# jbush001/RustNetworkStack

Hardware: AMD Instinct MI355X
Metric: GiB/s device-resident Internet checksum, 1500B-packet batches, 1/2/4/8 GPUs (higher is better)
Workload: dtype u8

## Files before the change

rustnetworkstack_amd/csrc/k_shapes.hip:

```cpp
#include "rns_launch.hpp"

namespace rns {

template <int G, int U, bool S>
int launch_shape(const CsumArgs &a, uint32_t variant, uint32_t max_blocks, hipStream_t st)
{
    uint64_t blocks;
    if ((variant & 5) == 0) {
        constexpr uint32_t kGroups = kBlock / G;
        blocks = (static_cast<uint64_t>(a.n) + kGroups - 1) / kGroups;
    } else {
        const uint64_t batches = waves64(a.n);
        const uint64_t wpb = ((variant & 4) ? kMixedBlock<false> : kBlock) / 64;
        blocks = (batches + wpb - 1) / wpb;
    }
    if (max_blocks != 0 && blocks > max_blocks)
        blocks = max_blocks;
    if (blocks == 0)
        return RNS_OK;
    const dim3 grid(static_cast<uint32_t>(blocks)), block((variant & 4) ? kMixedBlock<false> : kBlock);
    const bool nt = (variant & 2) != 0;
    const uint32_t cap = (variant >> 8) & 15u;
    const size_t lds = cap ? ((160u << 10) / cap) - (2u << 10) : 0u;
    variant &= 0xffu;
    if ((variant & 5) == 0) {
        if constexpr (G >= 4)
            return with_flags([&](auto NT) { return launch(csum_batch_kernel<G, U, S, NT()>, grid, block, lds, st, a); },
                              nt);
        return RNS_E_INVALID;
    }
    return with_flags(
        [&](auto NT, auto BUF) {
            if (variant & 4)
                return launch(csum_mixed_kernel<S, NT(), BUF(), false>, grid, block, lds, st, a);
            if constexpr (G <= 8 && U <= 2) {
                if (variant & 8)
                    return launch(csum_rounds_kernel<G, U, S, NT(), BUF(), G>, grid, block, lds, st, a);
                if (variant & 16)
                    return launch(csum_rounds_kernel<G, U, S, NT(), BUF(), 1, false, true>, grid, block, lds, st, a);
            } else if (variant & 24) {
                return static_cast<int>(RNS_E_INVALID);
            }
            return launch(csum_rounds_kernel<G, U, S, NT(), BUF()>, grid, block, lds, st, a);
        },
        nt, buf_ok(a));
}

template <bool S>
int dispatch(const CsumArgs &a, uint32_t variant, uint32_t G, uint32_t U, uint32_t max_blocks, hipStream_t st)
{
    const uint32_t v = variant & 0xffu;
    if (v > 31 || (variant >> 12) || ((v & 24) && (v & 5) != 1) || (v & 24) == 24)
        return RNS_E_INVALID;
    if (variant & 4)
        return launch_shape<64, 4, S>(a, variant, max_blocks, st);
#define RNS_SHAPE(g, u) \
    if (G == g && U == u) return launch_shape<g, u, S>(a, variant, max_blocks, st);
    if (variant & 1) {
        RNS_SHAPE(2, 1) RNS_SHAPE(2, 2) RNS_SHAPE(2, 4)
    }
    RNS_SHAPE(4, 1) RNS_SHAPE(4, 2) RNS_SHAPE(4, 4) RNS_SHAPE(4, 8)
    RNS_SHAPE(8, 1) RNS_SHAPE(8, 2) RNS_SHAPE(8, 4) RNS_SHAPE(8, 8)
    RNS_SHAPE(16, 1) RNS_SHAPE(16, 2) RNS_SHAPE(16, 4) RNS_SHAPE(16, 8)
    RNS_SHAPE(32, 1) RNS_SHAPE(32, 2) RNS_SHAPE(32, 4) RNS_SHAPE(32, 8)
    RNS_SHAPE(64, 1) RNS_SHAPE(64, 2) RNS_SHAPE(64, 4) RNS_SHAPE(64, 8)
#undef RNS_SHAPE
    return RNS_E_INVALID;
}

template int dispatch<false>(const CsumArgs &, uint32_t, uint32_t, uint32_t, uint32_t, hipStream_t);
template int dispatch<true>(const CsumArgs &, uint32_t, uint32_t, uint32_t, uint32_t, hipStream_t);

int launch_strided_tiny(const CsumArgs &a, hipStream_t st)
{
    constexpr int B = 2;
    const dim3 grid(static_cast<uint32_t>((static_cast<uint64_t>(a.n) + 64 * B - 1) / (64 * B))), block(64);
    return with_flags([&](auto buf) { return launch(csum_strided_tiny_kernel<buf(), B>, grid, block, 0, st, a); },
                      buf_ok(a));
}

}
```

rustnetworkstack_amd/csrc/rns_checksum.hip:

```cpp
#include <hip/hip_runtime.h>

#include <algorithm>
#include <cmath>
#include <cstdint>
#include <cstdio>

#include "rns_launch.hpp"

using namespace rns;

namespace {

__global__ __launch_bounds__(kBlock) void splitmix64_fill_kernel(uint8_t *buf, uint64_t nbytes, uint64_t seed)
{
    const uint64_t nwords = (nbytes + 7) / 8;
    const uint64_t stride = static_cast<uint64_t>(gridDim.x) * blockDim.x;
    for (uint64_t i = static_cast<uint64_t>(blockIdx.x) * blockDim.x + threadIdx.x; i < nwords; i += stride) {
        uint64_t z = seed + (i + 1) * 0x9E3779B97F4A7C15ull;
        z = (z ^ (z >> 30)) * 0xBF58476D1CE4E5B9ull;
        z = (z ^ (z >> 27)) * 0x94D049BB133111EBull;
        z = z ^ (z >> 31);
        if ((i + 1) * 8 <= nbytes) {
            reinterpret_cast<uint64_t *>(buf)[i] = z;
        } else {
            for (uint64_t b = i * 8; b < nbytes; ++b)
                buf[b] = static_cast<uint8_t>(z >> (8 * (b - i * 8)));
        }
    }
}

template <class Body>
int entry(uint32_t n, bool valid, const uint8_t *d_arena, uint64_t arena_bytes, uint32_t flags, void *stream, Body body)
{
    if (n == 0)
        return RNS_OK;
    if (!d_arena || !valid)
        return RNS_E_INVALID;
    if (int st = check_device())
        return st;
    CsumArgs a{};
    set_arena(a, d_arena, arena_bytes);
    a.n = n;
    a.flags = flags;
    return body(a, static_cast<hipStream_t>(stream));
}

void set_explicit(CsumArgs &a, const uint64_t *d_off, const uint32_t *d_len)
{
    a.off = d_off;
    a.len = d_len;
}

void set_packed(CsumArgs &a, const uint64_t *d_blk_off, const uint16_t *d_len16, uint32_t align_log2)
{
    a.len16 = d_len16;
    a.blk_off = d_blk_off;
    a.align_mask = (1u << align_log2) - 1u;
}

bool packed_align(uint32_t align_log2, uint32_t lo) { return align_log2 >= lo && align_log2 <= 12; }

void set_strided(CsumArgs &a, uint64_t first_off, uint64_t stride)
{
    a.first_off = first_off;
    a.stride = stride;
}

bool strided_fits(uint64_t first_off, uint64_t stride, uint32_t n)
{
    const uint64_t room = ~0ull - 16u - first_off;
    return first_off <= ~0ull - 16u && (n <= 1 || stride <= room / (n - 1));
}

void set_chain(CsumArgs &a, const uint64_t *d_frag_off, const uint32_t *d_frag_len, const uint32_t *d_first,
               uint32_t n_frags)
{
    a.off = d_frag_off;
    a.len = d_frag_len;
    a.first = d_first;
    a.n_frags = n_frags;
}

static_assert(RNS_CHAIN_MAX_PACKETS == 0xFFFFFFFFu - 64u * kChainMaxK, "rns_checksum.h's chain cap");
bool chain_valid(const uint64_t *d_frag_off, const uint32_t *d_frag_len, const uint32_t *d_first, uint32_t n_frags,
                 uint32_t n_pkts)
{
    return d_first && (!n_frags || (d_frag_off && d_frag_len)) && n_pkts <= RNS_CHAIN_MAX_PACKETS;
}

void set_results(CsumArgs &a, const uint16_t *d_seed, uint16_t *d_out, uint32_t *d_bad)
{
    a.seed = d_seed;
    a.out = d_out;
    a.bad = d_bad;
}

void set_field(CsumArgs &a, const uint16_t *d_field, uint32_t field_off)
{
    a.field = d_field;
    a.field_off = field_off;
}

uint32_t be_sum(const uint8_t *p, int nbytes)
{
    uint32_t s = 0;
    for (int k = 0; k < nbytes; k += 2)
        s += static_cast<uint32_t>(p[k]) << 8 | p[k + 1];
    return s;
}

void set_rx(CsumArgs &a, uint8_t *d_status, uint16_t *d_l4_sum, const uint8_t *local_ipv4, const uint8_t *local_ipv6)
{
    a.status = d_status;
    a.l4_out = d_l4_sum;
    a.local4_sum = be_sum(local_ipv4, 4);
    a.local6_sum = be_sum(local_ipv6, 16);
}

bool rx_valid(const uint8_t *d_status, const uint8_t *local_ipv4, const uint8_t *local_ipv6)
{
    return d_status && local_ipv4 && local_ipv6;
}

void set_tx_status(CsumArgs &a, uint8_t *d_status) { a.status = d_status; }

uint32_t chain_pick_k(double mean)
{
    uint32_t K = 1;
    double best = -1.0;
    for (uint32_t k = 1; k <= kChainMaxK; ++k) {
        const double fr = k * mean, fill = fr > 0 ? fr / std::ceil(fr) : 1.0;
        if (fill > best + 0.02) {
            best = fill;
            K = k;
        }
    }
    return K;
}

double chain_mean(const CsumArgs &a) { return static_cast<double>(a.n_frags) / static_cast<double>(a.n); }

#ifndef RNS_CHAIN_NT_FROM
#define RNS_CHAIN_NT_FROM 384u
#endif
bool chain_nt_from_hint(uint32_t frag_len_hint) { return (frag_len_hint ? frag_len_hint : 512u) >= RNS_CHAIN_NT_FROM; }
bool chain_nt_from_arena(uint64_t arena_bytes, uint32_t n_frags, double mean)
{
    const double frag_est = mean > 0.5 ? static_cast<double>(arena_bytes) / n_frags * (mean - 0.5) / mean : 0.0;
    return n_frags == 0 || frag_est >= RNS_CHAIN_NT_FROM;
}

bool chain_deep(uint32_t K, double mean) { return K >= 3 || (K == 2 && mean >= 2.0); }

template <bool FILL>
int chain_launch(CsumArgs &a, uint32_t frag_len_hint, hipStream_t stream)
{
    const double mean = chain_mean(a);
    a.chain_k = chain_pick_k(mean);
    if ((a.flags & RNS_FLAG_CHAIN_TX_PACKED) && mean <= 1.0 + kRunFrags)
        return launch_txrows<FILL>(a, stream);
    const bool runs = kChainRuns && (a.flags & RNS_FLAG_CHAIN_RUNS) && buf_ok(a);
    return launch_chain<FILL>(a, a.chain_k, chain_nt_from_hint(frag_len_hint), runs, chain_deep(a.chain_k, mean), stream);
}

constexpr uint64_t kRxGridCap = 4096;
dim3 stash_grid(uint64_t n, uint64_t arena_bytes, bool tiny_cap)
{
    constexpr int BLK = kMixedBlock<true>;
    uint64_t blocks = (waves64(n) + BLK / 64 - 1) / (BLK / 64);
    const bool cap = tiny_cap && arena_bytes / n <= 128;
    if (cap && blocks > kRxGridCap)
        blocks = kRxGridCap;
    return dim3(static_cast<uint32_t>(blocks));
}

}

extern "C" {

int rns_csum_batch_dev_cfg(const uint8_t *d_arena, uint64_t arena_bytes, const uint64_t *d_off,
                           const uint32_t *d_len, const uint16_t *d_seed, uint16_t *d_out, uint32_t n,
                           uint32_t flags, uint32_t variant, uint32_t lanes_per_packet, uint32_t unroll,
                           uint32_t max_blocks, uint32_t *d_bad, void *stream)
{
    return entry(n, d_off && d_len && d_out, d_arena, arena_bytes, flags, stream, [&](CsumArgs &a, hipStream_t st) {
        set_explicit(a, d_off, d_len);
        set_results(a, d_seed, d_out, d_bad);
        return dispatch<false>(a, variant, lanes_per_packet, unroll, max_blocks, st);
    });
}

int rns_csum_batch_dev(const uint8_t *d_arena, uint64_t arena_bytes, const uint64_t *d_off,
                       const uint32_t *d_len, const uint16_t *d_seed, uint16_t *d_out, uint32_t n,
                       uint32_t flags, uint32_t len_hint, uint32_t *d_bad, void *stream)
{
    const Shape sh = pick_shape(len_hint);
    return rns_csum_batch_dev_cfg(d_arena, arena_bytes, d_off, d_len, d_seed, d_out, n, flags, sh.variant, sh.G,
                                  sh.U, sh.max_blocks, d_bad, stream);
}

int rns_csum_batch_dev_off32(const uint8_t *d_arena, uint64_t arena_bytes, const uint32_t *d_off32,
                             const uint32_t *d_len, const uint16_t *d_seed, uint16_t *d_out, uint32_t n,
                             uint32_t flags, uint32_t len_hint, uint32_t *d_bad, void *stream)
{
    return entry(n, d_off32 && d_len && d_out, d_arena, arena_bytes, flags, stream, [&](CsumArgs &a, hipStream_t st) {
        a.off32 = d_off32;
        a.len = d_len;
        set_results(a, d_seed, d_out, d_bad);
        const Shape sh = pick_shape(len_hint);
        return dispatch<false>(a, sh.variant, sh.G, sh.U, sh.max_blocks, st);
    });
}

int rns_csum_batch_packed_dev(const uint8_t *d_arena, uint64_t arena_bytes, const uint64_t *d_blk_off,
                              const uint16_t *d_len16, uint32_t align_log2, const uint16_t *d_seed, uint16_t *d_out,
                              uint32_t n, uint32_t flags, uint32_t len_hint, uint32_t *d_bad, void *stream)
{
    return entry(n, d_blk_off && d_len16 && d_out && packed_align(align_log2, 0), d_arena, arena_bytes, flags, stream,
                 [&](CsumArgs &a, hipStream_t st) {
                     set_packed(a, d_blk_off, d_len16, align_log2);
                     set_results(a, d_seed, d_out, d_bad);
                     a.len_hint = len_hint;
                     Shape sh = pick_shape(len_hint);
                     if ((sh.variant & 5u) == 0)
                         sh = Shape{6u, 0u, 0u, 0u};
                     return dispatch_packed(a, sh, st);
                 });
}

int rns_csum_batch_strided_dev(const uint8_t *d_arena, uint64_t arena_bytes, uint64_t first_off,
                               uint64_t stride, uint32_t len, const uint16_t *d_seed, uint16_t *d_out,
                               uint32_t n, uint32_t flags, uint32_t *d_bad, void *stream)
{
    return entry(n, d_out && strided_fits(first_off, stride, n), d_arena, arena_bytes, flags, stream,
                 [&](CsumArgs &a, hipStream_t st) {
                     set_strided(a, first_off, stride);
                     set_results(a, d_seed, d_out, d_bad);
                     a.fixed_len = len;
                     if (len != 0 && len <= 64 && ((first_off + a.base_adjust) & 15) == 0 && (stride & 15) == 0)
                         return launch_strided_tiny(a, st);
                     const Shape sh = pick_shape(len);
                     return dispatch<true>(a, sh.variant, sh.G, sh.U, sh.max_blocks, st);
                 });
}

int rns_csum_chain_dev(const uint8_t *d_arena, uint64_t arena_bytes, const uint64_t *d_frag_off,
                       const uint32_t *d_frag_len, uint32_t n_frags, const uint32_t *d_first,
                       const uint16_t *d_seed, uint16_t *d_out, uint32_t n_pkts, uint32_t flags,
                       uint32_t frag_len_hint, uint16_t *d_frag_sums, uint32_t *d_bad, void *stream)
{
    (void)d_frag_sums;
    return entry(n_pkts, d_out && chain_valid(d_frag_off, d_frag_len, d_first, n_frags, n_pkts), d_arena, arena_bytes,
                 flags, stream, [&](CsumArgs &a, hipStream_t st) {
                     set_chain(a, d_frag_off, d_frag_len, d_first, n_frags);
                     set_results(a, d_seed, d_out, d_bad);
                     return chain_launch<false>(a, frag_len_hint, st);
                 });
}

int rns_csum_chain_fill_dev(uint8_t *d_arena, uint64_t arena_bytes, const uint64_t *d_frag_off,
                            const uint32_t *d_frag_len, uint32_t n_frags, const uint32_t *d_first,
                            const uint16_t *d_seed, const uint16_t *d_field, uint32_t field_off, uint16_t *d_out,
                            uint32_t n_pkts, uint32_t flags, uint32_t frag_len_hint, uint32_t *d_bad, void *stream)
{
    return entry(n_pkts, chain_valid(d_frag_off, d_frag_len, d_first, n_frags, n_pkts), d_arena, arena_bytes, flags,
                 stream, [&](CsumArgs &a, hipStream_t st) {
                     set_chain(a, d_frag_off, d_frag_len, d_first, n_frags);
                     set_results(a, d_seed, d_out, d_bad);
                     set_field(a, d_field, field_off);
                     return chain_launch<true>(a, frag_len_hint, st);
                 });
}

int rns_csum_fill_dev(uint8_t *d_arena, uint64_t arena_bytes, const uint64_t *d_off, const uint32_t *d_len,
                      const uint16_t *d_seed, const uint16_t *d_field, uint32_t field_off, uint16_t *d_out,
                      uint32_t n, uint32_t flags, uint32_t *d_bad, void *stream)
{
    return entry(n, d_off && d_len, d_arena, arena_bytes, flags, stream, [&](CsumArgs &a, hipStream_t st) {
        set_explicit(a, d_off, d_len);
        set_results(a, d_seed, d_out, d_bad);
        set_field(a, d_field, field_off);
        return launch_fill(a, stash_grid(n, arena_bytes, false), st);
    });
}

int rns_csum_fill_packed_dev(uint8_t *d_arena, uint64_t arena_bytes, const uint64_t *d_blk_off, const uint16_t *d_len16,
                             uint32_t align_log2, const uint16_t *d_seed, const uint16_t *d_field, uint32_t field_off,
                             uint16_t *d_out, uint32_t n, uint32_t flags, uint32_t len_hint, uint32_t *d_bad,
                             void *stream)
{
    return entry(n, d_blk_off && d_len16 && packed_align(align_log2, 4), d_arena, arena_bytes, flags, stream,
                 [&](CsumArgs &a, hipStream_t st) {
                     set_packed(a, d_blk_off, d_len16, align_log2);
                     set_results(a, d_seed, d_out, d_bad);
                     set_field(a, d_field, field_off);
                     a.len_hint = len_hint;
                     return launch_fill_packed(a, st);
                 });
}

int rns_rx_verify_dev(const uint8_t *d_arena, uint64_t arena_bytes, const uint64_t *d_off, const uint32_t *d_len,
                      uint32_t n, const uint8_t *local_ipv4, const uint8_t *local_ipv6, uint8_t *d_status,
                      uint16_t *d_l4_sum, void *stream)
{
    return entry(n, d_off && d_len && rx_valid(d_status, local_ipv4, local_ipv6), d_arena, arena_bytes,
                 RNS_FLAG_COMPLEMENT, stream, [&](CsumArgs &a, hipStream_t st) {
                     set_explicit(a, d_off, d_len);
                     set_rx(a, d_status, d_l4_sum, local_ipv4, local_ipv6);
                     return launch_rx(a, stash_grid(n, arena_bytes, true), st);
                 });
}

int rns_rx_verify_packed_dev(const uint8_t *d_arena, uint64_t arena_bytes, const uint64_t *d_blk_off,
                             const uint16_t *d_len16, uint32_t align_log2, uint32_t n, const uint8_t *local_ipv4,
                             const uint8_t *local_ipv6, uint8_t *d_status, uint16_t *d_l4_sum, void *stream)
{
    return entry(n, d_blk_off && d_len16 && rx_valid(d_status, local_ipv4, local_ipv6) && packed_align(align_log2, 4),
                 d_arena, arena_bytes, RNS_FLAG_COMPLEMENT, stream, [&](CsumArgs &a, hipStream_t st) {
                     set_packed(a, d_blk_off, d_len16, align_log2);
                     set_rx(a, d_status, d_l4_sum, local_ipv4, local_ipv6);
                     return launch_stream_rx(a, st);
                 });
}

int rns_rx_verify_strided_dev(const uint8_t *d_arena, uint64_t arena_bytes, uint64_t first_off, uint64_t stride,
                              const uint16_t *d_len16, uint32_t n, const uint8_t *local_ipv4, const uint8_t *local_ipv6,
                              uint8_t *d_status, uint16_t *d_l4_sum, void *stream)
{
    return entry(n, d_len16 && rx_valid(d_status, local_ipv4, local_ipv6) && strided_fits(first_off, stride, n), d_arena,
                 arena_bytes, RNS_FLAG_COMPLEMENT, stream, [&](CsumArgs &a, hipStream_t st) {
                     a.len16 = d_len16;
                     set_strided(a, first_off, stride);
                     set_rx(a, d_status, d_l4_sum, local_ipv4, local_ipv6);
                     return launch_strided_rx(a, st);
                 });
}

int rns_rx_verify_chain_dev(const uint8_t *d_arena, uint64_t arena_bytes, const uint64_t *d_frag_off,
                            const uint32_t *d_frag_len, uint32_t n_frags, const uint32_t *d_first, uint32_t n_pkts,
                            const uint8_t *local_ipv4, const uint8_t *local_ipv6, uint8_t *d_status, uint16_t *d_l4_sum,
                            void *stream)
{
    return entry(n_pkts,
                 chain_valid(d_frag_off, d_frag_len, d_first, n_frags, n_pkts) &&
                     rx_valid(d_status, local_ipv4, local_ipv6),
                 d_arena, arena_bytes, RNS_FLAG_COMPLEMENT, stream, [&](CsumArgs &a, hipStream_t st) {
                     set_chain(a, d_frag_off, d_frag_len, d_first, n_frags);
                     set_rx(a, d_status, d_l4_sum, local_ipv4, local_ipv6);
                     const double mean = chain_mean(a);
                     a.chain_k = chain_pick_k(mean);
                     return launch_rx_chain(a, a.chain_k, chain_nt_from_arena(arena_bytes, n_frags, mean), st);
                 });
}

int rns_rx_verify_pool_dev(const uint8_t *d_pool, uint64_t pool_bytes, uint32_t buf_log2, const uint32_t *d_buf_idx,
                           uint32_t n_frags, const uint32_t *d_blk_first, const uint16_t *d_len16, uint32_t n_pkts,
                           const uint8_t *local_ipv4, const uint8_t *local_ipv6, uint8_t *d_status, uint16_t *d_l4_sum,
                           void *stream)
{
    return entry(n_pkts,
                 buf_log2 >= kPoolMinLog2 && buf_log2 <= kPoolMaxLog2 && d_blk_first && d_len16 &&
                     (!n_frags || d_buf_idx) && n_pkts <= RNS_CHAIN_MAX_PACKETS &&
                     (reinterpret_cast<uintptr_t>(d_pool) & 15) == 0 && rx_valid(d_status, local_ipv4, local_ipv6),
                 d_pool, pool_bytes, RNS_FLAG_COMPLEMENT, stream, [&](CsumArgs &a, hipStream_t st) {
                     a.off32 = d_buf_idx;
                     a.n_frags = n_frags;
                     a.first = d_blk_first;
                     a.len16 = d_len16;
                     a.align_mask = (1u << buf_log2) - 1u;
                     set_rx(a, d_status, d_l4_sum, local_ipv4, local_ipv6);
                     const double mean = chain_mean(a);
                     a.chain_k = chain_pick_k(mean);
                     return launch_rx_pool(a, a.chain_k, chain_nt_from_arena(pool_bytes, n_frags, mean), st);
                 });
}

int rns_tx_fill_packed_dev(uint8_t *d_arena, uint64_t arena_bytes, const uint64_t *d_blk_off, const uint16_t *d_len16,
                           uint32_t align_log2, uint32_t n, uint8_t *d_status, uint32_t len_hint, void *stream)
{
    return entry(n, d_blk_off && d_len16 && packed_align(align_log2, 4), d_arena, arena_bytes, RNS_FLAG_COMPLEMENT,
                 stream, [&](CsumArgs &a, hipStream_t st) {
                     set_packed(a, d_blk_off, d_len16, align_log2);
                     set_tx_status(a, d_status);
                     a.len_hint = len_hint;
                     return launch_tx_packed(a, st);
                 });
}

int rns_tx_fill_chain_dev(uint8_t *d_arena, uint64_t arena_bytes, const uint64_t *d_frag_off, const uint32_t *d_frag_len,
                          uint32_t n_frags, const uint32_t *d_first, uint32_t n_pkts, uint8_t *d_status, void *stream)
{
    return entry(n_pkts, chain_valid(d_frag_off, d_frag_len, d_first, n_frags, n_pkts), d_arena, arena_bytes,
                 RNS_FLAG_COMPLEMENT, stream, [&](CsumArgs &a, hipStream_t st) {
                     set_chain(a, d_frag_off, d_frag_len, d_first, n_frags);
                     set_tx_status(a, d_status);
                     return launch_txrows<false, true>(a, st);
                 });
}

int rns_tx_fill_chain_packed_dev(uint8_t *d_arena, uint64_t arena_bytes, const uint64_t *d_head_blk_off,
                                 const uint8_t *d_head_len8, const uint64_t *d_pay_blk_off, const uint16_t *d_pay_len16,
                                 uint32_t pay_align_log2, uint32_t n, uint8_t *d_status, void *stream)
{
    return entry(n,
                 d_head_blk_off && d_head_len8 && d_pay_blk_off && d_pay_len16 && packed_align(pay_align_log2, 4) &&
                     n <= RNS_CHAIN_MAX_PACKETS,
                 d_arena, arena_bytes, RNS_FLAG_COMPLEMENT, stream, [&](CsumArgs &a, hipStream_t st) {
                     a.head_blk_off = d_head_blk_off;
                     a.head_len8 = d_head_len8;
                     set_packed(a, d_pay_blk_off, d_pay_len16, pay_align_log2);
                     set_tx_status(a, d_status);
                     return launch_txrows<false, true, true>(a, st);
                 });
}

int rns_tx_fill_dev(uint8_t *d_arena, uint64_t arena_bytes, const uint64_t *d_off, const uint32_t *d_len,
                    uint32_t n, uint8_t *d_status, void *stream)
{
    return entry(n, d_off && d_len, d_arena, arena_bytes, RNS_FLAG_COMPLEMENT, stream, [&](CsumArgs &a, hipStream_t st) {
        set_explicit(a, d_off, d_len);
        set_tx_status(a, d_status);
        return launch_tx(a, stash_grid(n, arena_bytes, true), st);
    });
}

int rns_fill_splitmix64_dev(uint8_t *d_buf, uint64_t nbytes, uint64_t seed, void *stream)
{
    if (nbytes == 0)
        return RNS_OK;
    if (!d_buf || (reinterpret_cast<uintptr_t>(d_buf) & 7))
        return RNS_E_INVALID;
    if (int st = check_device())
        return st;
    const uint64_t words = (nbytes + 7) / 8;
    const uint32_t blocks = static_cast<uint32_t>(std::min<uint64_t>((words + kBlock - 1) / kBlock, 8192));
    hipLaunchKernelGGL(splitmix64_fill_kernel, dim3(blocks), dim3(kBlock), 0, static_cast<hipStream_t>(stream),
                       d_buf, nbytes, seed);
    return hip_status(hipGetLastError());
}

const char *rns_csum_shape_name(uint32_t len_hint)
{
    static const char *const names[] = {"csum_batch_kernel",     "csum_rounds_kernel",     "csum_batch_kernel[nt]",
                                        "csum_rounds_kernel[nt]", "csum_mixed_kernel",      "csum_mixed_kernel",
                                        "csum_mixed_kernel[nt]",  "csum_mixed_kernel[nt]"};
    static thread_local char buf[96];
    const Shape sh = pick_shape(len_hint);
    if (sh.variant & 4)
        std::snprintf(buf, sizeof(buf), "%s (size classes G/U 4/1 x 4 packets, 4/4, 16/4, 32/4, 64/4)", names[sh.variant & 7]);
    else
        std::snprintf(buf, sizeof(buf), "%s<G=%u,U=%u>%s%s", names[sh.variant & 7], sh.G, sh.U,
                      (sh.variant & 8) ? " all rounds in flight" : (sh.variant & 16) ? " descriptors prefetched" : "",
                      sh.max_blocks ? " grid-capped" : "");
    return buf;
}

const char *rns_build_info(void)
{
    return "rns_checksum abi=1 offload-arch=gfx950 kernels=csum_rows_kernel (packed form: 1 KiB rows per 64-packet "
           "region, owners capture two region prefixes and sum their own end chunk; fill mode), csum_rows_rx_kernel "
           "(packed receive verify: the rows plus each owner's header chunks loaded a group ahead), csum_stream_kernel "
           "(receive verify of ACK-sized arenas: owners load their datagrams whole), csum_strided_rx_kernel (receive "
           "verify of fixed-size slots: quad-coalesced rows), csum_rows_tx_kernel (packed transmit finalize through the "
           "rows), csum_txrows_kernel (transmit-shaped chains: packed payload rows + owner-loaded head fragments; "
           "head-fragment fill; whole finalize of NetBuffer chains with the heads written back from LDS), "
           "csum_strided_tiny_kernel "
           "(fixed-size packets <= 64 B at a fixed stride), csum_mixed_kernel (per-wave size-class sort; verify / fill / "
           "transmit-finalize stash modes), csum_rounds_kernel, csum_batch_kernel, csum_chain_kernel (one pass, "
           "per-fragment fold; head-fragment fill) (v_sad_u16 LE sums, v_dot4 BE sums past 128 KiB, wave64, DPP "
           "reductions)";
}

int rns_device_count(void)
{
    int n = 0;
    if (hipGetDeviceCount(&n) != hipSuccess) {
        (void)hipGetLastError();
        return 0;
    }
    return n;
}

}
```

rustnetworkstack_amd/csrc/rns_kernels.hpp:

```cpp
#pragma once

#include "rns_k_common.hpp"
#include "rns_k_rounds.hpp"
#include "rns_k_mixed.hpp"
#include "rns_k_chain.hpp"
#include "rns_k_chain_rx.hpp"
#include "rns_k_pool_rx.hpp"
#include "rns_k_stream.hpp"
#include "rns_k_rows.hpp"
#include "rns_k_rows_rx.hpp"
#include "rns_k_rows_tx.hpp"
#include "rns_k_txrows.hpp"
```

rustnetworkstack_amd/csrc/rns_launch.hpp:

```cpp
#pragma once

#include <type_traits>

#include "rns_kernels.hpp"

namespace rns {

inline int hip_status(hipError_t e) { return e == hipSuccess ? RNS_OK : RNS_E_HIP_BASE - static_cast<int>(e); }

struct Shape {
    uint32_t variant, G, U, max_blocks;
};

constexpr uint32_t kTinyVariant = 19u;
constexpr uint32_t kTinyGrid = 2048u;
inline Shape pick_shape(uint32_t len_hint)
{
    const uint32_t chunks = len_hint ? (len_hint + 15) / 16 + 1 : 96;
    if (chunks <= 8)
        return Shape{kTinyVariant, 4u, 1u, kTinyGrid};
    if (chunks <= 48)
        return Shape{4u, 0u, 0u, 0u};
    if (chunks <= 160)
        return Shape{6u, 0u, 0u, 0u};
    return Shape{2u, 64u, 4u, 0u};
}

inline int check_device()
{
    int n = 0;
    if (hipGetDeviceCount(&n) != hipSuccess || n <= 0) {
        (void)hipGetLastError();
        return RNS_E_NODEVICE;
    }
    return RNS_OK;
}

inline void set_arena(CsumArgs &a, const uint8_t *arena, uint64_t arena_bytes)
{
    const uintptr_t p = reinterpret_cast<uintptr_t>(arena);
    a.base_adjust = p & 15;
    a.arena = reinterpret_cast<const uint8_t *>(p - a.base_adjust);
    a.arena_bytes = arena_bytes + a.base_adjust;
}

inline bool buf_ok(const CsumArgs &a) { return buf_records(a) < kOobOffset; }

inline uint32_t waves64(uint64_t n) { return static_cast<uint32_t>((n + 63) / 64); }

template <class F>
int with_flags(F &&f)
{
    return f();
}
template <class F, class... Rest>
int with_flags(F &&f, bool b, Rest... rest)
{
    auto bind = [&](auto c) { return with_flags([&](auto... cs) { return f(c, cs...); }, rest...); };
    return b ? bind(std::true_type{}) : bind(std::false_type{});
}

template <uint32_t KM, uint32_t... More, class F>
int with_kmax(uint32_t K, F &&f)
{
    if constexpr (sizeof...(More) == 0)
        return f(std::integral_constant<uint32_t, KM>{});
    else
        return K <= KM ? f(std::integral_constant<uint32_t, KM>{}) : with_kmax<More...>(K, f);
}

inline int launch(void (*kernel)(const CsumArgs), dim3 grid, dim3 block, size_t lds, hipStream_t st, const CsumArgs &a)
{
    hipLaunchKernelGGL(kernel, grid, block, lds, st, a);
    return hip_status(hipGetLastError());
}

template <bool S>
int dispatch(const CsumArgs &a, uint32_t variant, uint32_t G, uint32_t U, uint32_t max_blocks, hipStream_t st);
extern template int dispatch<false>(const CsumArgs &, uint32_t, uint32_t, uint32_t, uint32_t, hipStream_t);
extern template int dispatch<true>(const CsumArgs &, uint32_t, uint32_t, uint32_t, uint32_t, hipStream_t);
int launch_strided_tiny(const CsumArgs &a, hipStream_t st);
int dispatch_packed(const CsumArgs &a, const Shape &sh, hipStream_t st);
int launch_fill_packed(const CsumArgs &a, hipStream_t st);
int launch_stream_rx(const CsumArgs &a, hipStream_t st);
int launch_tx_packed(const CsumArgs &a, hipStream_t st);
int launch_strided_rx(const CsumArgs &a, hipStream_t st);
template <bool FILL>
int launch_chain(const CsumArgs &a, uint32_t K, bool nt, bool runs, bool deep, hipStream_t st);
extern template int launch_chain<false>(const CsumArgs &, uint32_t, bool, bool, bool, hipStream_t);
extern template int launch_chain<true>(const CsumArgs &, uint32_t, bool, bool, bool, hipStream_t);
template <bool FILL, bool FIN = false, bool CPT = false>
int launch_txrows(const CsumArgs &a, hipStream_t st);
extern template int launch_txrows<false, false, false>(const CsumArgs &, hipStream_t);
extern template int launch_txrows<true, false, false>(const CsumArgs &, hipStream_t);
extern template int launch_txrows<false, true, false>(const CsumArgs &, hipStream_t);
extern template int launch_txrows<false, true, true>(const CsumArgs &, hipStream_t);
int launch_rx_chain(const CsumArgs &a, uint32_t K, bool nt, hipStream_t st);
int launch_rx_pool(const CsumArgs &a, uint32_t K, bool nt, hipStream_t st);
int launch_fill(const CsumArgs &a, dim3 grid, hipStream_t st);
int launch_rx(const CsumArgs &a, dim3 grid, hipStream_t st);
int launch_tx(const CsumArgs &a, dim3 grid, hipStream_t st);

}
```

rustnetworkstack_amd/csrc/rns_pipeline.hip:

```cpp
#include <hip/hip_runtime.h>

#include <algorithm>
#include <cstdint>
#include <cstring>
#include <mutex>
#include <new>
#include <thread>
#include <vector>

#include "rns_launch.hpp"

using namespace rns;

struct rns_host_ctx {
    struct Slot {
        hipStream_t stream = nullptr;
        hipEvent_t done = nullptr;
        uint8_t *d_arena = nullptr;
        uint64_t *d_off = nullptr;
        uint32_t *d_len = nullptr;
        uint16_t *d_seed = nullptr;
        uint16_t *d_out = nullptr;
        uint64_t *h_off = nullptr;
        uint32_t *h_len = nullptr;
        uint16_t *h_seed = nullptr;
        uint16_t *h_out = nullptr;
        bool busy = false;
        uint32_t i0 = 0, cnt = 0;
    };
    int device = 0;
    uint64_t chunk_bytes = 0;
    uint32_t chunk_packets = 0;
    std::vector<Slot> slots;
    std::mutex mu;
};

namespace {

void free_ctx(rns_host_ctx *c)
{
    if (!c)
        return;
    (void)hipSetDevice(c->device);
    for (auto &s : c->slots) {
        if (s.stream) (void)hipStreamSynchronize(s.stream);
        if (s.done) (void)hipEventDestroy(s.done);
        if (s.stream) (void)hipStreamDestroy(s.stream);
        (void)hipFree(s.d_arena); (void)hipFree(s.d_off); (void)hipFree(s.d_len);
        (void)hipFree(s.d_seed); (void)hipFree(s.d_out);
        (void)hipHostFree(s.h_off); (void)hipHostFree(s.h_len);
        (void)hipHostFree(s.h_seed); (void)hipHostFree(s.h_out);
    }
    delete c;
}

int drain_slot(rns_host_ctx::Slot &s, uint16_t *h_out)
{
    if (!s.busy)
        return RNS_OK;
    s.busy = false;
    int st = hip_status(hipEventSynchronize(s.done));
    if (st == RNS_OK)
        std::memcpy(h_out + s.i0, s.h_out, static_cast<size_t>(s.cnt) * sizeof(uint16_t));
    return st;
}

}

extern "C" {

int rns_host_ctx_create(int device, uint64_t chunk_bytes, uint32_t nstreams, rns_host_ctx **out)
{
    if (!out || nstreams == 0 || nstreams > 16 || chunk_bytes < 4096)
        return RNS_E_INVALID;
    *out = nullptr;
    if (int st = check_device())
        return st;
    int st = hip_status(hipSetDevice(device));
    if (st)
        return st;
    rns_host_ctx *c = new (std::nothrow) rns_host_ctx;
    if (!c)
        return RNS_E_INVALID;
    c->device = device;
    c->chunk_bytes = (chunk_bytes + 255) & ~255ull;
    c->chunk_packets = static_cast<uint32_t>(std::min<uint64_t>(c->chunk_bytes / 16, 1u << 24));
    c->slots.resize(nstreams);
    const size_t np = c->chunk_packets;
    for (auto &s : c->slots) {
        hipError_t e = hipSuccess;
        if (e == hipSuccess) e = hipStreamCreateWithFlags(&s.stream, hipStreamNonBlocking);
        if (e == hipSuccess) e = hipEventCreateWithFlags(&s.done, hipEventDisableTiming);
        if (e == hipSuccess) e = hipMalloc(reinterpret_cast<void **>(&s.d_arena), c->chunk_bytes + 256);
        if (e == hipSuccess) e = hipMalloc(reinterpret_cast<void **>(&s.d_off), np * sizeof(uint64_t));
        if (e == hipSuccess) e = hipMalloc(reinterpret_cast<void **>(&s.d_len), np * sizeof(uint32_t));
        if (e == hipSuccess) e = hipMalloc(reinterpret_cast<void **>(&s.d_seed), np * sizeof(uint16_t));
        if (e == hipSuccess) e = hipMalloc(reinterpret_cast<void **>(&s.d_out), np * sizeof(uint16_t));
        if (e == hipSuccess) e = hipHostMalloc(reinterpret_cast<void **>(&s.h_off), np * sizeof(uint64_t), 0);
        if (e == hipSuccess) e = hipHostMalloc(reinterpret_cast<void **>(&s.h_len), np * sizeof(uint32_t), 0);
        if (e == hipSuccess) e = hipHostMalloc(reinterpret_cast<void **>(&s.h_seed), np * sizeof(uint16_t), 0);
        if (e == hipSuccess) e = hipHostMalloc(reinterpret_cast<void **>(&s.h_out), np * sizeof(uint16_t), 0);
        if (e != hipSuccess) {
            free_ctx(c);
            return hip_status(e);
        }
    }
    *out = c;
    return RNS_OK;
}

int rns_host_ctx_destroy(rns_host_ctx *ctx)
{
    free_ctx(ctx);
    return RNS_OK;
}

int rns_csum_batch_host(rns_host_ctx *ctx, const uint8_t *h_arena, uint64_t arena_bytes,
                        const uint64_t *h_off, const uint32_t *h_len, const uint16_t *h_seed,
                        uint16_t *h_out, uint32_t n, uint32_t flags)
{
    if (!ctx)
        return RNS_E_INVALID;
    if (n == 0)
        return RNS_OK;
    if (!h_arena || !h_off || !h_len || !h_out)
        return RNS_E_INVALID;
    for (uint32_t i = 0; i < n; ++i) {
        if (h_off[i] > arena_bytes || h_len[i] > arena_bytes - h_off[i])
            return RNS_E_BOUNDS;
        if (i && h_off[i] < h_off[i - 1])
            return RNS_E_ORDER;
        if ((h_off[i] & 255u) + h_len[i] > ctx->chunk_bytes)
            return RNS_E_TOOLARGE;
    }
    std::lock_guard<std::mutex> lock(ctx->mu);
    int st = hip_status(hipSetDevice(ctx->device));
    if (st)
        return st;
    const size_t nslots = ctx->slots.size();
    size_t k = 0;
    uint32_t i0 = 0;
    while (i0 < n && st == RNS_OK) {
        const uint64_t lo = h_off[i0] & ~255ull;
        uint64_t hi = lo;
        uint32_t i1 = i0;
        while (i1 < n && i1 - i0 < ctx->chunk_packets) {
            const uint64_t end = std::max(hi, h_off[i1] + h_len[i1]);
            if (end - lo > ctx->chunk_bytes)
                break;
            hi = end;
            ++i1;
        }
        if (i1 == i0) {
            st = RNS_E_TOOLARGE;
            break;
        }
        auto &s = ctx->slots[k++ % nslots];
        st = drain_slot(s, h_out);
        if (st)
            break;
        const uint32_t cnt = i1 - i0;
        std::memcpy(s.h_off, h_off + i0, cnt * sizeof(uint64_t));
        std::memcpy(s.h_len, h_len + i0, cnt * sizeof(uint32_t));
        if (h_seed)
            std::memcpy(s.h_seed, h_seed + i0, cnt * sizeof(uint16_t));
        hipError_t e = hipMemcpyAsync(s.d_arena, h_arena + lo, hi - lo, hipMemcpyHostToDevice, s.stream);
        if (e == hipSuccess) e = hipMemcpyAsync(s.d_off, s.h_off, cnt * sizeof(uint64_t), hipMemcpyHostToDevice, s.stream);
        if (e == hipSuccess) e = hipMemcpyAsync(s.d_len, s.h_len, cnt * sizeof(uint32_t), hipMemcpyHostToDevice, s.stream);
        if (e == hipSuccess && h_seed)
            e = hipMemcpyAsync(s.d_seed, s.h_seed, cnt * sizeof(uint16_t), hipMemcpyHostToDevice, s.stream);
        if (e != hipSuccess) {
            st = hip_status(e);
            break;
        }
        CsumArgs a{};
        a.arena = s.d_arena - lo;
        a.arena_bytes = hi;
        a.base_adjust = 0;
        a.off = s.d_off;
        a.len = s.d_len;
        a.seed = h_seed ? s.d_seed : nullptr;
        a.out = s.d_out;
        a.n = cnt;
        a.flags = flags;
        const Shape sh = pick_shape(static_cast<uint32_t>(std::min<uint64_t>((hi - lo) / cnt, 1u << 30)));
        st = dispatch<false>(a, sh.variant, sh.G, sh.U, sh.max_blocks, s.stream);
        if (st)
            break;
        e = hipMemcpyAsync(s.h_out, s.d_out, cnt * sizeof(uint16_t), hipMemcpyDeviceToHost, s.stream);
        if (e == hipSuccess) e = hipEventRecord(s.done, s.stream);
        if (e != hipSuccess) {
            st = hip_status(e);
            break;
        }
        s.busy = true;
        s.i0 = i0;
        s.cnt = cnt;
        i0 = i1;
    }
    for (auto &s : ctx->slots) {
        int d = drain_slot(s, h_out);
        if (st == RNS_OK)
            st = d;
    }
    return st;
}

struct rns_multi_ctx {
    std::vector<rns_host_ctx *> ctx;
};

int rns_multi_ctx_create(const int *devices, uint32_t ndev, uint64_t chunk_bytes, uint32_t nstreams,
                         rns_multi_ctx **out)
{
    if (!out || !devices || ndev == 0 || ndev > 64)
        return RNS_E_INVALID;
    *out = nullptr;
    rns_multi_ctx *m = new (std::nothrow) rns_multi_ctx;
    if (!m)
        return RNS_E_INVALID;
    for (uint32_t i = 0; i < ndev; ++i) {
        rns_host_ctx *c = nullptr;
        const int st = rns_host_ctx_create(devices[i], chunk_bytes, nstreams, &c);
        if (st) {
            rns_multi_ctx_destroy(m);
            return st;
        }
        m->ctx.push_back(c);
    }
    *out = m;
    return RNS_OK;
}

int rns_multi_ctx_destroy(rns_multi_ctx *ctx)
{
    if (ctx) {
        for (rns_host_ctx *c : ctx->ctx)
            rns_host_ctx_destroy(c);
        delete ctx;
    }
    return RNS_OK;
}

extern "C++" {
namespace {
std::vector<uint32_t> split_by_bytes(const uint32_t *len, uint32_t n, uint32_t parts)
{
    uint64_t total = 0;
    for (uint32_t i = 0; i < n; ++i)
        total += len[i];
    std::vector<uint32_t> bounds(parts + 1, n);
    bounds[0] = 0;
    uint64_t acc = 0;
    uint32_t i = 0;
    for (uint32_t k = 1; k < parts; ++k) {
        const uint64_t target = total * k / parts;
        while (i < n && acc + len[i] <= target)
            acc += len[i++];
        bounds[k] = std::max(i, bounds[k - 1]);
    }
    return bounds;
}
}
}

int rns_csum_batch_multi_host(rns_multi_ctx *ctx, const uint8_t *h_arena, uint64_t arena_bytes,
                              const uint64_t *h_off, const uint32_t *h_len, const uint16_t *h_seed,
                              uint16_t *h_out, uint32_t n, uint32_t flags)
{
    if (!ctx || ctx->ctx.empty())
        return RNS_E_INVALID;
    if (n == 0)
        return RNS_OK;
    if (!h_arena || !h_off || !h_len || !h_out)
        return RNS_E_INVALID;
    const uint32_t parts = static_cast<uint32_t>(ctx->ctx.size());
    const std::vector<uint32_t> b = split_by_bytes(h_len, n, parts);
    std::vector<int> st(parts, RNS_OK);
    auto run = [&](uint32_t k) {
        const uint32_t i0 = b[k], cnt = b[k + 1] - b[k];
        if (cnt)
            st[k] = rns_csum_batch_host(ctx->ctx[k], h_arena, arena_bytes, h_off + i0, h_len + i0,
                                        h_seed ? h_seed + i0 : nullptr, h_out + i0, cnt, flags);
    };
    std::vector<std::thread> workers;
    for (uint32_t k = 1; k < parts; ++k) {
        try {
            workers.emplace_back(run, k);
        } catch (...) {
            run(k);
        }
    }
    run(0);
    for (auto &w : workers)
        w.join();
    for (int x : st)
        if (x)
            return x;
    return RNS_OK;
}

int rns_csum_batch_multi_dev(const rns_dev_batch *batches, uint32_t nbatches, uint32_t flags)
{
    if (nbatches == 0)
        return RNS_OK;
    if (!batches)
        return RNS_E_INVALID;
    if (int st = check_device())
        return st;
    int prev = 0;
    if (hipGetDevice(&prev) != hipSuccess)
        return RNS_E_NODEVICE;
    int st = RNS_OK;
    for (uint32_t k = 0; k < nbatches && st == RNS_OK; ++k) {
        const rns_dev_batch &d = batches[k];
        st = hip_status(hipSetDevice(d.device));
        if (st == RNS_OK)
            st = rns_csum_batch_dev(d.d_arena, d.arena_bytes, d.d_off, d.d_len, d.d_seed, d.d_out, d.n, flags,
                                    d.len_hint, d.d_bad, d.stream);
    }
    (void)hipSetDevice(prev);
    return st;
}

int rns_host_alloc(uint64_t bytes, void **out)
{
    if (!out)
        return RNS_E_INVALID;
    *out = nullptr;
    if (int st = check_device())
        return st;
    return hip_status(hipHostMalloc(out, bytes, 0));
}

int rns_host_free(void *p) { return hip_status(hipHostFree(p)); }

}
```

Measured before the change: 6732.

## Stream ascending 16-byte-aligned explicit-descriptor waves as contiguous rows

Adds a new kernel for explicit-descriptor batches. When one wave's 64 packets start on 16-byte boundaries and sit in ascending order, with little padding between them, the wave reads the whole region as contiguous 1 KiB rows and credits each row segment to its packet. Other waves fall back to the size-class pass. This targets the scattered per-packet loads of the mixed-size path for contiguously laid-out 1500B batches, at the cost of a per-wave scan and ballot to detect the layout, plus a one-wave block shape.

```diff
diff --git a/rustnetworkstack_amd/csrc/k_shapes.hip b/rustnetworkstack_amd/csrc/k_shapes.hip
--- a/rustnetworkstack_amd/csrc/k_shapes.hip
+++ b/rustnetworkstack_amd/csrc/k_shapes.hip
@@ -71,6 +71,23 @@
 template int dispatch<false>(const CsumArgs &, uint32_t, uint32_t, uint32_t, uint32_t, hipStream_t);
 template int dispatch<true>(const CsumArgs &, uint32_t, uint32_t, uint32_t, uint32_t, hipStream_t);
 
+constexpr int kRowsXImixD = 8;
+int launch_explicit(const CsumArgs &a, uint32_t len_hint, hipStream_t st)
+{
+    const Shape sh = pick_shape(len_hint);
+    if ((sh.variant & 4u) == 0)
+        return dispatch<false>(a, sh.variant, sh.G, sh.U, sh.max_blocks, st);
+    if (a.n == 0)
+        return RNS_OK;
+    const dim3 grid(waves64(a.n)), block(64);
+    return with_flags(
+        [&](auto mtu, auto buf) {
+            constexpr int D = mtu() ? 16 : kRowsXImixD;
+            return launch(csum_rows_x_kernel<mtu(), buf(), D, 4>, grid, block, 0, st, a);
+        },
+        (sh.variant & 2u) != 0, buf_ok(a));
+}
+
 int launch_strided_tiny(const CsumArgs &a, hipStream_t st)
 {
     constexpr int B = 2;
diff --git a/rustnetworkstack_amd/csrc/rns_checksum.hip b/rustnetworkstack_amd/csrc/rns_checksum.hip
--- a/rustnetworkstack_amd/csrc/rns_checksum.hip
+++ b/rustnetworkstack_amd/csrc/rns_checksum.hip
@@ -194,9 +194,11 @@
                        const uint32_t *d_len, const uint16_t *d_seed, uint16_t *d_out, uint32_t n,
                        uint32_t flags, uint32_t len_hint, uint32_t *d_bad, void *stream)
 {
-    const Shape sh = pick_shape(len_hint);
-    return rns_csum_batch_dev_cfg(d_arena, arena_bytes, d_off, d_len, d_seed, d_out, n, flags, sh.variant, sh.G,
-                                  sh.U, sh.max_blocks, d_bad, stream);
+    return entry(n, d_off && d_len && d_out, d_arena, arena_bytes, flags, stream, [&](CsumArgs &a, hipStream_t st) {
+        set_explicit(a, d_off, d_len);
+        set_results(a, d_seed, d_out, d_bad);
+        return launch_explicit(a, len_hint, st);
+    });
 }
 
 int rns_csum_batch_dev_off32(const uint8_t *d_arena, uint64_t arena_bytes, const uint32_t *d_off32,
@@ -207,8 +209,7 @@
         a.off32 = d_off32;
         a.len = d_len;
         set_results(a, d_seed, d_out, d_bad);
-        const Shape sh = pick_shape(len_hint);
-        return dispatch<false>(a, sh.variant, sh.G, sh.U, sh.max_blocks, st);
+        return launch_explicit(a, len_hint, st);
     });
 }
 
@@ -444,10 +445,13 @@
     static const char *const names[] = {"csum_batch_kernel",     "csum_rounds_kernel",     "csum_batch_kernel[nt]",
                                         "csum_rounds_kernel[nt]", "csum_mixed_kernel",      "csum_mixed_kernel",
                                         "csum_mixed_kernel[nt]",  "csum_mixed_kernel[nt]"};
-    static thread_local char buf[96];
+    static thread_local char buf[320];
     const Shape sh = pick_shape(len_hint);
     if (sh.variant & 4)
-        std::snprintf(buf, sizeof(buf), "%s (size classes G/U 4/1 x 4 packets, 4/4, 16/4, 32/4, 64/4)", names[sh.variant & 7]);
+        std::snprintf(buf, sizeof(buf),
+                      "csum_rows_x_kernel (explicit descriptors: a wave whose 64 packets ascend at 16-byte starts "
+                      "streams them as 1 KiB rows; any other wave runs the %s size-class pass, G/U 4/1 x 4 packets, "
+                      "4/4, 16/4, 32/4, 64/4)", names[sh.variant & 7]);
     else
         std::snprintf(buf, sizeof(buf), "%s<G=%u,U=%u>%s%s", names[sh.variant & 7], sh.G, sh.U,
                       (sh.variant & 8) ? " all rounds in flight" : (sh.variant & 16) ? " descriptors prefetched" : "",
@@ -465,7 +469,8 @@
            "rows), csum_txrows_kernel (transmit-shaped chains: packed payload rows + owner-loaded head fragments; "
            "head-fragment fill; whole finalize of NetBuffer chains with the heads written back from LDS), "
            "csum_strided_tiny_kernel "
-           "(fixed-size packets <= 64 B at a fixed stride), csum_mixed_kernel (per-wave size-class sort; verify / fill / "
+           "(fixed-size packets <= 64 B at a fixed stride), csum_rows_x_kernel (explicit descriptors: the rows for "
+           "every wave whose packets ascend at 16-byte starts, the class pass for the others), csum_mixed_kernel (per-wave size-class sort; verify / fill / "
            "transmit-finalize stash modes), csum_rounds_kernel, csum_batch_kernel, csum_chain_kernel (one pass, "
            "per-fragment fold; head-fragment fill) (v_sad_u16 LE sums, v_dot4 BE sums past 128 KiB, wave64, DPP "
            "reductions)";
diff --git a/rustnetworkstack_amd/csrc/rns_k_rows_x.hpp b/rustnetworkstack_amd/csrc/rns_k_rows_x.hpp
--- /dev/null
+++ b/rustnetworkstack_amd/csrc/rns_k_rows_x.hpp
@@ -0,0 +1,59 @@
+#pragma once
+
+#include "rns_k_stream.hpp"
+
+namespace rns {
+
+template <bool NT, bool BUF, int D, int OCC>
+__global__ __launch_bounds__(64, OCC) void csum_rows_x_kernel(const CsumArgs a)
+{
+    constexpr bool kRowsNT = RNS_STREAM_NT != 0;
+    const uint32_t lane = threadIdx.x;
+    const __amdgpu_buffer_rsrc_t rsrc = __builtin_amdgcn_make_buffer_rsrc(
+        const_cast<uint8_t *>(a.arena), static_cast<short>(0), static_cast<int>(BUF ? buf_records(a) : 0), 0x00020000);
+    const uint64_t recs = buf_records(a);
+    const uint64_t p = static_cast<uint64_t>(blockIdx.x) * 64 + lane;
+    const bool live = p < a.n;
+    const Desc<BUF> cd = load_desc<false, false, BUF>(a, p);
+    uint64_t d_start = cd.off + a.base_adjust;
+    uint32_t d_len = cd.len;
+    const uint32_t d_seed = (a.seed && live) ? a.seed[p] : 0u;
+    const bool d_ok = d_start <= a.arena_bytes && d_len <= a.arena_bytes - d_start;
+    const bool has = live && d_ok && d_len != 0;
+    if (!has) {
+        d_len = 0;
+        d_start = 0;
+    }
+    const uint64_t hm = __ballot(has);
+    bool region = false;
+    uint64_t r0 = 0;
+    uint32_t rel = 0, total = 0;
+    if (hm) {
+        r0 = lane_u64(d_start, static_cast<uint32_t>(__builtin_ctzll(hm)));
+        const uint64_t rel64 = has ? d_start - r0 : 0;
+        const bool fits = has && (d_start & 15u) == 0 && rel64 < (1ull << 30) && d_len <= kNoWrapBytes;
+        const uint32_t pad = fits ? (d_len + 15u) & ~15u : 0u;
+        rel = static_cast<uint32_t>(rel64);
+        const uint32_t incl = wave_incl_max(fits ? rel + pad : 0u);
+        const uint32_t before = static_cast<uint32_t>(__shfl(static_cast<int>(incl), static_cast<int>(lane) - 1, 64));
+        const bool asc = !has || (fits && (lane == 0 || rel >= before));
+        total = __builtin_amdgcn_readlane(incl, 63);
+        const uint32_t sum_pad = __builtin_amdgcn_readlane(wave_incl_scan(pad), 63);
+        region = !__ballot(!asc) && total <= 2u * sum_pad + 4096u;
+    }
+    uint32_t mine = 0;
+    if (region) {
+        const uint32_t c0 = has ? rel >> 4 : 0u;
+        const uint32_t e = has ? (rel + d_len - 1u) >> 4 : 0u;
+        mine = rows_region_sum<kRowsNT, BUF, D>(a, rsrc, recs, r0, total, c0, e, d_len);
+    } else if (hm) {
+        uint32_t pos;
+        mine = wave_class_pass<NT, BUF, kStashNone>(a, rsrc, d_start, d_len, 0xFFFFFFFFu, lane, nullptr, pos);
+    }
+    const uint16_t res = finalize_bits(mine, d_start & 1, d_len > kNoWrapBytes, d_seed, d_ok, a.flags);
+    if (live && a.out)
+        __builtin_nontemporal_store(res, a.out + p);
+    count_rejected(a, lane, live && !d_ok);
+}
+
+}
diff --git a/rustnetworkstack_amd/csrc/rns_kernels.hpp b/rustnetworkstack_amd/csrc/rns_kernels.hpp
--- a/rustnetworkstack_amd/csrc/rns_kernels.hpp
+++ b/rustnetworkstack_amd/csrc/rns_kernels.hpp
@@ -11,3 +11,4 @@
 #include "rns_k_rows_rx.hpp"
 #include "rns_k_rows_tx.hpp"
 #include "rns_k_txrows.hpp"
+#include "rns_k_rows_x.hpp"
diff --git a/rustnetworkstack_amd/csrc/rns_launch.hpp b/rustnetworkstack_amd/csrc/rns_launch.hpp
--- a/rustnetworkstack_amd/csrc/rns_launch.hpp
+++ b/rustnetworkstack_amd/csrc/rns_launch.hpp
@@ -80,6 +80,7 @@
 extern template int dispatch<false>(const CsumArgs &, uint32_t, uint32_t, uint32_t, uint32_t, hipStream_t);
 extern template int dispatch<true>(const CsumArgs &, uint32_t, uint32_t, uint32_t, uint32_t, hipStream_t);
 int launch_strided_tiny(const CsumArgs &a, hipStream_t st);
+int launch_explicit(const CsumArgs &a, uint32_t len_hint, hipStream_t st);
 int dispatch_packed(const CsumArgs &a, const Shape &sh, hipStream_t st);
 int launch_fill_packed(const CsumArgs &a, hipStream_t st);
 int launch_stream_rx(const CsumArgs &a, hipStream_t st);
diff --git a/rustnetworkstack_amd/csrc/rns_pipeline.hip b/rustnetworkstack_amd/csrc/rns_pipeline.hip
--- a/rustnetworkstack_amd/csrc/rns_pipeline.hip
+++ b/rustnetworkstack_amd/csrc/rns_pipeline.hip
@@ -183,8 +183,7 @@
         a.out = s.d_out;
         a.n = cnt;
         a.flags = flags;
-        const Shape sh = pick_shape(static_cast<uint32_t>(std::min<uint64_t>((hi - lo) / cnt, 1u << 30)));
-        st = dispatch<false>(a, sh.variant, sh.G, sh.U, sh.max_blocks, s.stream);
+        st = launch_explicit(a, static_cast<uint32_t>(std::min<uint64_t>((hi - lo) / cnt, 1u << 30)), s.stream);
         if (st)
             break;
         e = hipMemcpyAsync(s.h_out, s.d_out, cnt * sizeof(uint16_t), hipMemcpyDeviceToHost, s.stream);
```

After: 6732. Within noise of the previous version (-0.0%).
